# firedrakeproject/fiat

Hardware: AMD Instinct MI355X
Metric: element tabulations/sec (basis+grad, fp64) for batched P3 tet (higher is better)
Workload: dtype f64; 1 GPU; Lagrange degree 3 tetrahedron, order 1, 23 points/request, batch 100000 per GPU; requests_per_gpu=100000, points_per_request=23, order=1, points=random per request, world_size=1, launch=single process, clock_ramp_steps=224

## Files before the change

fiat_amd/csrc/api.hip:

```cpp
#include <hip/hip_runtime.h>

#include <algorithm>
#include <cmath>
#include <cstdarg>
#include <cstdio>
#include <cstring>
#include <cstdlib>
#include <mutex>
#include <string>
#include <thread>
#include <numeric>
#include <vector>

#include "../../include/fiat_amd.h"
#include "aux_kernels.hpp"
#include "plan.hpp"
#include "simplex_kernel.hpp"
#include "simplex_fixed.hpp"
#include "simplex_stream.hpp"
#include "simplex_pair.hpp"
#include "coop_kernel.hpp"
#include "shared_points.hpp"
#include "quadrature.hpp"
#include "simplex_small.hpp"
// ... 489 lines not shown

int fx_element_create(fx_ctx* ctx, int sd, int n, int variant, double scale, const double* verts,
                      int ndof, int vdim, const double* coeffs, fx_element** out) {
    if (!ctx || !out) return fail(FX_EINVAL, "fx_element_create: null argument");
    if (sd < 1 || sd > 3) return fail(FX_EINVAL, "Invalid number of spatial dimensions");
    if (n < 0) return fail(FX_EINVAL, "negative degree");
    if (variant < 0 || variant > 2) return fail(FX_EINVAL, "Invalid variant %d", variant);
    if (variant == FX_VARIANT_BUBBLE && n < 1) return fail(FX_EINVAL, "bubble variant needs degree >= 1");
    if (ndof < 1 || vdim < 1) return fail(FX_EINVAL, "bad ndof/vdim");
    HIP_TRY(hipSetDevice(ctx->device));
    fx_element* e = new fx_element;
    e->ctx = ctx;
    e->sd = sd;
    e->n = n;
    e->variant = variant;
    e->nexp = fx::binom(n + sd, sd);
    if (scale <= 0.0) {
        scale = std::sqrt(1.0 / default_simplex_volume(sd));
        if (n == 0 && sd > 1) scale = 1.0;
    }
    e->scale = scale;
    if (!host_cell_map(sd, verts ? verts : UFC[sd - 1], e->A0, e->b0)) {
        delete e;
        return fail(FX_EINVAL, "degenerate cell");
    }
    e->prog = fx::build_program(sd, n, variant, scale);
    if (variant == FX_VARIANT_BUBBLE) e->T = fx::c0_transform(sd, n);
    static_assert(sizeof(fx::Step) == sizeof(fxk::Step), "step layout");
    size_t sbytes = std::max<size_t>(1, e->prog.steps.size()) * sizeof(fxk::Step);
    hipError_t he = hipMalloc(&e->d_steps, sbytes);
    if (he == hipSuccess && !e->prog.steps.empty())
        he = hipMemcpy(e->d_steps, e->prog.steps.data(), e->prog.steps.size() * sizeof(fxk::Step), hipMemcpyHostToDevice);
    if (he != hipSuccess) {
        fx_element_destroy(e);
        return fail(FX_EHIP, "fx_element_create: %s", hipGetErrorString(he));
    }
    int rc = upload_coeffs(e, ndof, vdim, coeffs);
    if (rc != FX_OK) {
        fx_element_destroy(e);
        return rc;
    }
    *out = e;
    return FX_OK;
}

int fx_element_destroy(fx_element* e) {
    if (!e) return FX_OK;
    if (e->d_steps) (void)hipFree(e->d_steps);
    if (e->d_cmat) (void)hipFree(e->d_cmat);
    if (e->d_afrag) (void)hipFree(e->d_afrag);
    if (e->d_afrag_split) (void)hipFree(e->d_afrag_split);
    if (e->d_afrag_stream) (void)hipFree(e->d_afrag_stream);
    if (e->d_coop_eint) (void)hipFree(e->d_coop_eint);
    if (e->d_coop_edbl) (void)hipFree(e->d_coop_edbl);
    if (e->d_coop_kstart) (void)hipFree(e->d_coop_kstart);
    if (e->d_afrag_coop) (void)hipFree(e->d_afrag_coop);
    for (int o = 0; o < 3; ++o)
        if (e->d_astack[o]) (void)hipFree(e->d_astack[o]);
    for (int o = 0; o < 3; ++o) {
        if (e->d_astack_dm[o]) (void)hipFree(e->d_astack_dm[o]);
        if (e->d_astack_dmp[o]) (void)hipFree(e->d_astack_dmp[o]);
    }
    for (int o = 0; o <= FX_MAX_ORDER; ++o)
        if (e->high[o]) fx_element_destroy(e->high[o]);
    delete e;
    return FX_OK;
}

int fx_element_set_coeffs(fx_element* e, int ndof, int vdim, const double* coeffs) {
    if (!e || ndof < 1 || vdim < 1) return fail(FX_EINVAL, "fx_element_set_coeffs: bad argument");
    HIP_TRY(hipSetDevice(e->ctx->device));
    return upload_coeffs(e, ndof, vdim, coeffs);
}

int fx_element_dims(const fx_element* e, int* sd, int* n, int* nexp, int* ndof, int* vdim) {
    if (!e) return fail(FX_EINVAL, "fx_element_dims: null element");
    if (sd) *sd = e->sd;
    if (n) *n = e->n;
    if (nexp) *nexp = e->nexp;
    if (ndof) *ndof = e->ndof;
    if (vdim) *vdim = e->vdim;
    return FX_OK;
}

}

namespace {

struct Launch {
    fxk::TabArgs args;
    int grid = 0, lds_bytes = 0;
    int fixed_id = -1;
    fxk::FixedArgs<0> fhead;
    std::vector<double> fcoef;
    std::vector<double> fucoef;
    int fgrid = 0, flds_bytes = 0, ncu = 0;
    bool fused_mapping = false;
    bool kodd = false;
    int kpiola = 0;
    double* trash = nullptr;
    fx_ctx* ctx = nullptr;
    int fkind = 0;
    int small_id = -1;
    fxk::SmallArgs sargs;
    int sgrid = 0, slds_bytes = 0;
    int stacked_id = -1;
    fxk::StackedArgs<0> khead;
    int kgrid = 0, klds_bytes = 0, kmix_order = 0;
    int wg_ct = 0;
    int wg_mix = 0;
    int coop_id = -1;
    fxk::CoopArgs cargs;
    int cgrid = 0, clds_bytes = 0;
};

constexpr int FIXED_NW = 4;
struct FixedShape {
    int sd, n, order, rows, nt;
    bool pair_only;
    int rpw;
    bool fullimg;
    int nw;
    bool can_piola;
};
const FixedShape kFixedShapes[] = {
    {3, 3, 1, 20, 6, false, 2, true, 8, false},
    {3, 3, 1, 20, 5, true, 2, true, 8, false},
    {3, 3, 1, 20, 4, true, 2, true, 8, false},
    {3, 3, 1, 20, 3, true, 2, true, 8, false},
    {3, 3, 1, 20, 8, true, 1, false, 8, false},
    {3, 3, 1, 20, 10, true, 1, false, 8, false},
    {3, 3, 1, 20, 12, true, 1, false, 8, false},
    {3, 2, 1, 45, 6, true, 1, false, 8, true},
    {3, 4, 1, 35, 6, true, 1, false, 8, false},
    {3, 2, 1, 60, 6, true, 1, false, 4, true},
    {3, 3, 0, 20, 2, true, 2, true, 8, false},
    {3, 3, 0, 20, 3, true, 1, true, 8, false},
    {3, 4, 0, 35, 2, true, 2, true, 8, false},
    {3, 4, 0, 35, 3, true, 1, true, 8, false},
};

template <int SD, int N>
bool table_matches(const fx::Program& P) {
    constexpr fxk::StepTable<SD, N> T{};
    if ((int)P.steps.size() != T.count) return false;
    for (int i = 0; i < T.count; ++i)
        if (P.steps[i].dst != T.dst[i] || P.steps[i].cur != T.cur[i] || P.steps[i].prv != T.prv[i] ||
            P.steps[i].codim != T.codim[i])
            return false;
    return true;
}

#if defined(FX_DBG) && (FX_DBG & 512)
hipError_t report_wave_lifetimes(const double* trash, int grid, int wg_waves) {
    const int nw = std::min(grid * wg_waves, 3000);
    std::vector<double> t(2 * nw);
    hipError_t e = hipDeviceSynchronize();
    if (e != hipSuccess) return e;
    e = hipMemcpy(t.data(), trash + 2048, t.size() * 8, hipMemcpyDeviceToHost);
    if (e != hipSuccess) return e;
    std::vector<double> us(nw), mhz(nw);
    for (int i = 0; i < nw; ++i) {
        us[i] = t[2 * i + 1] / 100.0;
        mhz[i] = t[2 * i] / us[i];
    }
    std::vector<double> su = us, sm = mhz;
    std::sort(su.begin(), su.end());
    std::sort(sm.begin(), sm.end());
    fprintf(stderr, "[fiat_amd] %d waves: lifetime us min %.1f p10 %.1f median %.1f p90 %.1f max %.1f | clock MHz min %.0f median %.0f max %.0f\n",
            nw, su[0], su[nw / 10], su[nw / 2], su[nw * 9 / 10], su[nw - 1], sm[0], sm[nw / 2], sm[nw - 1]);
    for (int x = 0; x < 8; ++x) {
        std::vector<double> v;
        for (int i = 0; i < nw; ++i)
            if (((i / wg_waves) % 8) == x) v.push_back(us[i]);
        if (v.empty()) continue;
        std::sort(v.begin(), v.end());
        fprintf(stderr, " xcd%d %.0f..%.0f..%.0f", x, v[0], v[v.size() / 2], v.back());
    }
    {
        std::vector<double> ab(2 * nw), ini(nw);
        if (hipMemcpy(ab.data(), trash + 2048 + 6000, ab.size() * 8, hipMemcpyDeviceToHost) == hipSuccess &&
            hipMemcpy(ini.data(), trash + 2048 + 12000, ini.size() * 8, hipMemcpyDeviceToHost) == hipSuccess) {
            double t0 = 1e300, t1 = 0;
            for (int i = 0; i < nw; ++i) {
                t0 = std::min(t0, ab[2 * i]);
                t1 = std::max(t1, ab[2 * i + 1]);
            }
            std::vector<double> st(nw), en(nw);
            for (int i = 0; i < nw; ++i) {
                st[i] = (ab[2 * i] - t0) / 100.0;
                en[i] = (t1 - ab[2 * i + 1]) / 100.0;
            }
            std::vector<double> ss = st, se = en, si = ini;
            std::sort(ss.begin(), ss.end());
            std::sort(se.begin(), se.end());
            std::sort(si.begin(), si.end());
            fprintf(stderr, "\n span %.1f us | entry after first entry: p50 %.1f p90 %.1f max %.1f us | init->first unit: p50 %.1f max %.1f us | idle before the last exit: p10 %.1f p50 %.1f p90 %.1f max %.1f us (mean %.1f)",
                    (t1 - t0) / 100.0, ss[nw / 2], ss[nw * 9 / 10], ss[nw - 1], si[nw / 2] / 100.0, si[nw - 1] / 100.0, se[nw / 10], se[nw / 2],
                    se[nw * 9 / 10], se[nw - 1], std::accumulate(se.begin(), se.end(), 0.0) / nw);
            for (int x = 0; x < 8; ++x) {
                double ms = 0, me = 0;
                int n = 0;
                for (int i = 0; i < nw; ++i)
                    if (((i / wg_waves) % 8) == x) ms += st[i], me += en[i], ++n;
                if (n) fprintf(stderr, "%s xcd%d entry +%.1f idle-at-end %.1f", x == 0 ? "\n" : " |", x, ms / n, me / n);
            }
        }
    }
    fprintf(stderr, "\n workgroup lifetimes (max over its waves), XCD0:");
    for (int b = 0; b < grid; b += 8) {
        double m = 0;
        for (int w = 0; w < wg_waves && b * wg_waves + w < nw; ++w) m = std::max(m, us[b * wg_waves + w]);
        fprintf(stderr, " %.0f", m);
    }
    fprintf(stderr, "\n");
    return hipSuccess;
}
#endif

#ifndef FX_PAIR_BALANCE
#define FX_PAIR_BALANCE 0
#endif
template <int SD, int N, int ORDER, int ROWS, int NT, bool PAIR_ONLY = false, int RPW = 2, bool FULLIMG = true, int PAIR_NW = 8,
          bool CAN_PIOLA = false>
int launch_fixed(const Launch& L, hipStream_t s) {
    using KernT = void (*)(const fxk::FixedArgs<fxk::FixedNC<SD, N>::value>);
    constexpr int NC = fxk::FixedNC<SD, N>::value;
    fxk::FixedArgs<NC> fa;
    fa.pts = L.fhead.pts;
    fa.verts = L.fhead.verts;
    fa.out = L.fhead.out;
    fa.afrag = L.fhead.afrag;
    fa.phi0 = L.fhead.phi0;
    memcpy(fa.A0, L.fhead.A0, sizeof fa.A0);
    memcpy(fa.b0, L.fhead.b0, sizeof fa.b0);
    fa.nreq = L.fhead.nreq;
    fa.npts = L.fhead.npts;
    fa.lds_doubles = L.fhead.lds_doubles;
    fa.debug = L.fhead.debug;
    if ((int)L.fcoef.size() != NC || (int)L.fucoef.size() != 4 * NC)
        return fail(FX_EINVAL, "internal: coefficient table size mismatch");
    memcpy(fa.coef, L.fcoef.data(), NC * sizeof(double));
    memcpy(fa.ucoef, L.fucoef.data(), 4 * NC * sizeof(double));
    if (L.fkind == 2) {
        using KernP = void (*)(const fxk::FixedArgs<NC>, double*, unsigned int*);
        KernP kp = L.fhead.verts ? (KernP)fxk::tabulate_simplex_pair<SD, N, ORDER, ROWS, NT, PAIR_NW, false, RPW, FULLIMG>
                                 : (KernP)fxk::tabulate_simplex_pair<SD, N, ORDER, ROWS, NT, PAIR_NW, true, RPW, FULLIMG>;
        if ((fa.debug >> 16) & 3) {
            if constexpr (CAN_PIOLA) kp = (KernP)fxk::tabulate_simplex_pair<SD, N, ORDER, ROWS, NT, PAIR_NW, false, RPW, FULLIMG, true>;
            else return fail(FX_EINVAL, "internal: no fused push-forward for this shape");
        }
        const int lds_bytes = fxk::WQ_CTL_DOUBLES * 8 + (L.flds_bytes - (int)(fa.lds_doubles * 8) * FIXED_NW) + (int)(fa.lds_doubles * 8) * PAIR_NW;
        static thread_local const void* cached_kp = nullptr;
        static thread_local int cached_lds = -1, cached_occ = 0;
        if (cached_kp != reinterpret_cast<const void*>(kp) || cached_lds != lds_bytes) {
            if (lds_bytes > 48 * 1024)
                HIP_TRY(hipFuncSetAttribute(reinterpret_cast<const void*>(kp), hipFuncAttributeMaxDynamicSharedMemorySize, lds_bytes));
            int q = 0;
            HIP_TRY(hipOccupancyMaxActiveBlocksPerMultiprocessor(&q, reinterpret_cast<const void*>(kp), 64 * PAIR_NW, (size_t)lds_bytes));
            cached_kp = reinterpret_cast<const void*>(kp);
            cached_lds = lds_bytes;
            cached_occ = q;
        }
        const int occ = cached_occ;
        const long long nwg = ((L.fhead.nreq + RPW - 1) / RPW + PAIR_NW - 1) / PAIR_NW;
        int grid = (int)std::max<long long>(1, std::min<long long>(nwg, (long long)L.ncu * std::max(1, occ)));
#if FX_PAIR_BALANCE
        if (nwg > grid) {
            long long best = (nwg + grid - 1) / grid * grid - nwg;
            for (int g = grid - 1; g >= grid - grid / 8 && best > 0; --g) {
                const long long waste = (nwg + g - 1) / g * g - nwg;
                if (waste < best) {
                    best = waste;
                    grid = g;
                }
            }
        }
#endif
        static const bool verbose = ab_env("FIAT_AMD_VERBOSE") != nullptr;
        if (verbose) fprintf(stderr, "[fiat_amd] pair kernel: occupancy %d WG/CU, grid %d, lds %d B\n", occ, grid, lds_bytes);
        unsigned int* const counter = work_counter(L.ctx, s);
        if (!counter) return FX_ENOMEM;
        hipLaunchKernelGGL(kp, dim3(grid), dim3(64 * PAIR_NW), lds_bytes, s, fa, L.trash, counter);
        HIP_TRY(hipGetLastError());
#if defined(FX_DBG) && (FX_DBG & 512)
        if (verbose) HIP_TRY(report_wave_lifetimes(L.trash, grid, PAIR_NW));
#endif
        return FX_OK;
    }
    if constexpr (PAIR_ONLY) {
        return fail(FX_EINVAL, "internal: only the paired kernel exists for this shape");
    } else {
        KernT kern;
        if (L.fkind == 1)
            kern = L.fhead.verts ? (KernT)fxk::tabulate_simplex_stream<SD, N, ORDER, ROWS, NT, FIXED_NW, false>
                                 : (KernT)fxk::tabulate_simplex_stream<SD, N, ORDER, ROWS, NT, FIXED_NW, true>;
        else
            kern = (KernT)fxk::tabulate_simplex_fixed<SD, N, ORDER, ROWS, NT, FIXED_NW>;
        if (L.flds_bytes > 48 * 1024)
            HIP_TRY(hipFuncSetAttribute(reinterpret_cast<const void*>(kern), hipFuncAttributeMaxDynamicSharedMemorySize,
                                        L.flds_bytes));
        const int grid = L.fgrid;
        hipLaunchKernelGGL(kern, dim3(grid), dim3(64 * FIXED_NW), L.flds_bytes, s, fa);
        HIP_TRY(hipGetLastError());
        return FX_OK;
    }
}

struct StackedShape {
    int sd, n, ct, g;
    int rtc;
};
const StackedShape kStackedShapes[] = {
    {3, 3, 3, 2, 5},
    {3, 3, 2, 1, 5},
    {3, 3, 3, 1, 5},
    {3, 6, 2, 1, -2}, {3, 5, 3, 2, -2}, {3, 5, 2, 1, -2}, {3, 5, 3, 1, -2},
    {2, 6, 3, 2, -2}, {2, 6, 2, 1, -2}, {2, 6, 3, 1, -2}, {2, 5, 3, 2, -2}, {2, 5, 2, 1, -2}, {2, 5, 3, 1, -2},
    {3, 4, 3, 2, -2}, {3, 4, 2, 1, -2}, {3, 4, 3, 1, -2}, {3, 3, 3, 2, -2}, {3, 3, 2, 1, -2}, {3, 3, 3, 1, -2},
    {3, 6, 3, 2, 0},
    {3, 6, 2, 1, 0},
    {3, 6, 3, 1, 0},
    {3, 5, 3, 2, 0},
    {3, 5, 2, 1, 0},
    {3, 5, 3, 1, 0},
    {3, 4, 3, 2, 0},
    {3, 4, 2, 1, 0},
    {3, 4, 3, 1, 0},
    {3, 3, 3, 2, 0},
    {3, 3, 2, 1, 0},
    {3, 3, 3, 1, 0},
    {2, 6, 3, 2, 0},
    {2, 6, 2, 1, 0},
    {2, 6, 3, 1, 0},
    {2, 5, 3, 2, 0},
    {2, 5, 2, 1, 0},
    {2, 5, 3, 1, 0},
    {3, 6, 3, 3, 0},
    {3, 5, 3, 3, 0}, {3, 5, 4, 1, 0},
    {3, 4, 3, 3, 0}, {3, 4, 4, 1, 0},
    {3, 3, 3, 3, 0}, {3, 3, 4, 1, 0},
    {2, 6, 3, 3, 0}, {2, 6, 4, 1, 0},
    {2, 5, 3, 3, 0}, {2, 5, 4, 1, 0},
    {3, 2, 3, 2, 0}, {3, 2, 2, 1, 0}, {3, 2, 3, 1, 0}, {3, 2, 3, 3, 0}, {3, 2, 4, 1, 0},
    {3, 6, 3, 1, -1}, {3, 5, 3, 1, -1}, {3, 4, 3, 1, -1}, {3, 3, 3, 1, -1}, {3, 2, 3, 1, -1}, {2, 6, 3, 1, -1}, {2, 5, 3, 1, -1},
    {3, 2, 3, 4, 0},
    {2, 4, 3, 3, 0}, {2, 4, 3, 2, 0}, {2, 4, 2, 1, 0}, {2, 4, 3, 1, 0},
    {2, 3, 3, 4, 0}, {2, 3, 3, 3, 0}, {2, 3, 3, 2, 0}, {2, 3, 2, 1, 0},
    {3, 2, 3, 6, 0}, {3, 2, 3, 8, 0}, {3, 2, 3, 12, 0},
    {2, 3, 3, 6, 0}, {2, 3, 3, 8, 0}, {2, 4, 3, 4, 0}, {2, 4, 3, 6, 0},
    {2, 4, 3, 1, -1}, {2, 3, 3, 1, -1},
    {3, 2, 3, 4, -2}, {3, 2, 3, 3, -2}, {3, 2, 3, 2, -2}, {3, 2, 2, 1, -2},
    {2, 3, 3, 4, -2}, {2, 3, 3, 3, -2}, {2, 3, 3, 2, -2}, {2, 4, 3, 3, -2}, {2, 4, 3, 2, -2}, {2, 4, 2, 1, -2},
    {3, 7, 2, 1, 0}, {3, 7, 2, 1, -1},
    {2, 7, 3, 1, 0}, {2, 7, 2, 1, 0}, {2, 7, 3, 1, -1}, {2, 8, 4, 1, 0}, {2, 8, 3, 1, -1},
    {3, 2, 3, 4, -3}, {3, 2, 3, 3, -3}, {3, 2, 3, 2, -3}, {3, 2, 2, 1, -3},
    {3, 3, 3, 2, -3}, {3, 3, 2, 1, -3}, {3, 3, 3, 1, -3},
    {3, 4, 3, 2, -3}, {3, 4, 2, 1, -3}, {3, 4, 3, 1, -3},
    {3, 5, 2, 1, -3}, {3, 6, 2, 1, -3},
    {2, 3, 3, 4, -3}, {2, 3, 3, 3, -3}, {2, 3, 3, 2, -3},
    {2, 4, 3, 3, -3}, {2, 4, 3, 2, -3}, {2, 4, 2, 1, -3},
    {2, 5, 3, 2, -3}, {2, 5, 2, 1, -3}, {2, 5, 3, 1, -3},
    {2, 6, 3, 2, -3}, {2, 6, 2, 1, -3}, {2, 6, 3, 1, -3},
    {3, 6, 3, 2, -2}, {3, 6, 3, 1, -2},
    {3, 6, 3, 1, -4}, {3, 5, 3, 1, -4}, {3, 4, 3, 1, -4}, {3, 3, 3, 1, -4}, {3, 2, 3, 1, -4}, {2, 6, 3, 1, -4}, {2, 5, 3, 1, -4},
    {3, 6, 2, 1, -5}, {3, 5, 2, 1, -5}, {3, 4, 2, 1, -5}, {3, 3, 3, 1, -5}, {3, 2, 3, 1, -5}, {2, 6, 3, 1, -5}, {2, 5, 3, 1, -5},
    {3, 2, 3, 4, -6}, {3, 2, 3, 3, -6}, {3, 2, 3, 2, -6}, {3, 2, 2, 1, -6}, {3, 3, 3, 2, -6}, {3, 3, 2, 1, -6}, {3, 3, 3, 1, -6},
    {2, 3, 3, 4, -6}, {2, 3, 3, 3, -6}, {2, 3, 3, 2, -6}, {2, 4, 3, 3, -6}, {2, 4, 3, 2, -6}, {2, 4, 2, 1, -6},
    {3, 6, 2, 1, -1}, {3, 5, 2, 1, -1},
    {3, 6, 2, 1, -4}, {3, 5, 2, 1, -4},
    {3, 6, 8, 1, -7}, {3, 5, 8, 1, -7}, {3, 4, 8, 1, -7}, {3, 3, 8, 1, -7}, {2, 6, 8, 1, -7}, {2, 5, 8, 1, -7},
};
constexpr bool stacked_has_pio(int sd, int n) { return (sd == 3 && (n == 2 || n == 3)) || (sd == 2 && (n == 3 || n == 4)); }
constexpr int STACKED_NW = 4;
#ifndef FX_MIXR1
#define FX_MIXR1 1
#endif
constexpr bool mixr1(int sd, int n, int ct, int g) {
    return FX_MIXR1 == 2 || (FX_MIXR1 != 0 && !(sd == 2 && g == 1 && n == 4 && ct == 2));
}
constexpr int mixr_wps(int sd, int n) { return sd == 2 && n >= 5 ? 2 : 1; }
template <int SD>
int stacked_mix_pass(const Launch& L, hipStream_t s) {
    if (L.khead.verts && L.kmix_order >= 1) {
        fxk::TableMixArgs ma;
        ma.out = L.khead.out;
        ma.verts = L.khead.verts;
        if (!invert_small(SD, L.khead.A0, ma.A0inv)) return fail(FX_EINVAL, "degenerate cell");
        const int ntab = fx::binom(SD + L.kmix_order, SD);
        ma.n = L.khead.R / ntab * L.khead.npts;
        ma.order = L.kmix_order;
        ma.slices = std::max(1, std::min(8, (ma.n + 2047) / 2048));
        ma.nreq = L.khead.nreq;
        ma.rb = ma.n >= 1024 ? 1 : std::max(1, std::min(fxk::MIX_RB, 2048 / std::max(1, ma.n)));
        if (L.khead.nreq * ma.slices > 0x7fffffffLL) return fail(FX_EINVAL, "batch too large for the table-mixing pass");
        if ((long long)fxk::MIX_RB * ma.n > 0x3fffffffLL) return fail(FX_EINVAL, "request too large for the table-mixing pass");
        const long long blocks = ma.rb > 1 ? std::min<long long>((L.khead.nreq + ma.rb - 1) / ma.rb, (long long)L.ncu * 16) : L.khead.nreq * ma.slices;
        hipLaunchKernelGGL((fxk::table_mix_kernel<SD>), dim3((unsigned)std::max<long long>(1, blocks)), dim3(256), 0, s, ma);
        HIP_TRY(hipGetLastError());
    }
    return FX_OK;
}

template <int SD, int N, int CT, int G, int RTC = 0, int WPS = 1, bool CHUNK = false, int MIXT = 0, bool ODD = false, bool MIXR = false, int PIO = 0>
int launch_stacked(const Launch& L, hipStream_t s) {
    constexpr int NC = fxk::FixedNC<SD, N>::value;
    fxk::StackedArgs<NC> ka;
    ka.pts = L.khead.pts;
    ka.verts = L.khead.verts;
    ka.out = L.khead.out;
    ka.afrag = L.khead.afrag;
    ka.phi0 = L.khead.phi0;
    memcpy(ka.A0, L.khead.A0, sizeof ka.A0);
    memcpy(ka.b0, L.khead.b0, sizeof ka.b0);
    memcpy(ka.A0inv, L.khead.A0inv, sizeof ka.A0inv);
    memcpy(ka.G, L.khead.G, sizeof ka.G);
    ka.piola = L.khead.piola;
    ka.nreq = L.khead.nreq;
    ka.npts = L.khead.npts;
    ka.R = L.khead.R;
    ka.RT = L.khead.RT;
    ka.debug = L.khead.debug;
    ka.lim_pts = L.khead.lim_pts;
    ka.lim_verts = L.khead.lim_verts;
    ka.lim_out = L.khead.lim_out;
    ka.lim_afrag = L.khead.lim_afrag;
    if ((int)L.fcoef.size() != NC) return fail(FX_EINVAL, "internal: coefficient table size mismatch");
    memcpy(ka.coef, L.fcoef.data(), NC * sizeof(double));
    auto kern = fxk::tabulate_simplex_stacked<SD, N, CT, G, RTC, WPS, CHUNK, MIXT, ODD, MIXR, PIO>;
    static thread_local int occ = 0;
    if (occ == 0) {
        if (L.klds_bytes > 48 * 1024)
            HIP_TRY(hipFuncSetAttribute(reinterpret_cast<const void*>(kern), hipFuncAttributeMaxDynamicSharedMemorySize, L.klds_bytes));
        int q = 0;
        HIP_TRY(hipOccupancyMaxActiveBlocksPerMultiprocessor(&q, reinterpret_cast<const void*>(kern), 64 * STACKED_NW, (size_t)L.klds_bytes));
        occ = std::max(1, q);
        static const int cap = ab_env("FIAT_AMD_STACKED_WPS") ? atoi(ab_env("FIAT_AMD_STACKED_WPS")) : 8;
        occ = std::min(occ, std::max(1, cap));
        if (ab_env("FIAT_AMD_VERBOSE")) fprintf(stderr, "[fiat_amd] stacked kernel <%d,%d,%d,%d>: %d workgroups per CU, lds %d B\n", SD, N, CT, G, occ, L.klds_bytes);
// ... 2698 lines not shown
```

fiat_amd/csrc/simplex_pair.hpp:

```cpp
#pragma once
#include "simplex_stream.hpp"
#include "work_queue.hpp"

#ifndef FX_DBG
#define FX_DBG 0
#endif
#ifndef FX_PAIR_FULLIMG
#define FX_PAIR_FULLIMG 1
#endif
#ifndef FX_PAIR_PLAIN_EDGES
#define FX_PAIR_PLAIN_EDGES 1
#endif
#ifndef FX_PAIR_WAVES
#define FX_PAIR_WAVES 2
#endif

namespace fxk {

template <int SD, int N, int ORDER, int ROWS, int NT, int NW, bool UNIFORM, int RPW = 2, bool FULLIMG = (FX_PAIR_FULLIMG != 0),
          bool PIOLA = false>
__global__ __launch_bounds__(64 * NW, NW <= 4 ? 1 : FX_PAIR_WAVES) void tabulate_simplex_pair(const FixedArgs<FixedNC<SD, N>::value> a,
                                                                                double* __restrict__ trash,
                                                                                unsigned int* __restrict__ gqueue) {
    constexpr int NTAB = NTab<SD, ORDER>::value;
    constexpr StepTable<SD, N> TBL{};
    constexpr int NEXP = StepTable<SD, N>::NEXP;
    constexpr int KS = (NEXP + 3) / 4;
    constexpr int MT16 = rows_full16(ROWS);
    constexpr int M4 = rows_blk4(ROWS);
    static_assert(RPW == 1 || RPW == 2, "one or two requests per wave");
    static_assert(!PIOLA || (!UNIFORM && ROWS % SD == 0), "the Piola map needs per-request cells and SD components per dof");
    constexpr int NT2 = RPW * NT;
    extern __shared__ __attribute__((aligned(16))) double lds[];
    const int lane = threadIdx.x & 63;
    const int wave = __builtin_amdgcn_readfirstlane((int)(threadIdx.x >> 6));
#if FX_DBG & 512
    const unsigned long long rt_entry = __builtin_amdgcn_s_memrealtime();
#endif
    constexpr int NAF = (MT16 + M4) * KS;
    double* afr = lds + WQ_CTL_DOUBLES;
    double* img = afr + NAF * 64 + (size_t)wave * a.lds_doubles;
    double* slab = img;
    const int dump = a.lds_doubles - 64;

    typedef const __attribute__((address_space(4))) double CDouble;
    typedef FixedArgs<FixedNC<SD, N>::value> ArgsT;
    const __attribute__((address_space(4))) char* kargs =
        (const __attribute__((address_space(4))) char*)__builtin_amdgcn_kernarg_segment_ptr();
    CDouble* kcoef = (CDouble*)(kargs + __builtin_offsetof(ArgsT, coef));
    CDouble* kucoef = (CDouble*)(kargs + __builtin_offsetof(ArgsT, ucoef));

    const int npts = a.npts;
    double a0inv[SD][SD];
    if constexpr (PIOLA) {
        if constexpr (SD == 2) {
            const double det = a.A0[0] * a.A0[3] - a.A0[1] * a.A0[2];
            a0inv[0][0] = a.A0[3] / det;
            a0inv[0][1] = -a.A0[1] / det;
            a0inv[1][0] = -a.A0[2] / det;
            a0inv[1][1] = a.A0[0] / det;
        } else {
            const double* A = a.A0;
            const double c00 = A[4] * A[8] - A[5] * A[7], c01 = A[5] * A[6] - A[3] * A[8], c02 = A[3] * A[7] - A[4] * A[6];
            const double det = A[0] * c00 + A[1] * c01 + A[2] * c02;
            a0inv[0][0] = c00 / det;
            a0inv[0][1] = (A[2] * A[7] - A[1] * A[8]) / det;
            a0inv[0][2] = (A[1] * A[5] - A[2] * A[4]) / det;
            a0inv[1][0] = c01 / det;
            a0inv[1][1] = (A[0] * A[8] - A[2] * A[6]) / det;
            a0inv[1][2] = (A[2] * A[3] - A[0] * A[5]) / det;
            a0inv[2][0] = c02 / det;
            a0inv[2][1] = (A[1] * A[6] - A[0] * A[7]) / det;
            a0inv[2][2] = (A[0] * A[4] - A[1] * A[3]) / det;
        }
    }
    const int table = ROWS * npts;

    for (int i = lane; i < a.lds_doubles; i += 64) img[i] = 0.0;
    for (int i = threadIdx.x; i < NAF * 64; i += 64 * NW) afr[i] = a.afrag[i];
    const long long npairs = (a.nreq + RPW - 1) / RPW;
#ifndef FX_WQ_TAIL
#define FX_WQ_TAIL 0
#endif
    WorkQueueT<(FX_WQ_TAIL != 0)> wqueue;
    wqueue.init(lds, gqueue, npairs);
    __syncthreads();

    const int sub = RPW == 2 ? lane >> 5 : 0;
    const int lp = RPW == 2 ? lane & 31 : lane;
    const bool active = lp < npts;
    const int pl = active ? lp : 0;
    static_assert(FULLIMG || NT % 2 == 0 || NTAB == 1, "half-aligned column tiles need an even tile count");
    constexpr int TH = FULLIMG ? NTAB : (NTAB + 1) / 2;
    constexpr int NTH = NTAB > TH ? NT / 2 : NT;
    int colbase[NTAB];
#pragma unroll
    for (int t = 0; t < NTAB; ++t) {
        const int h = t >= TH ? 1 : 0;
        const int c = (t - h * TH) * npts + pl;
        colbase[t] = active ? (sub * NT + h * NTH + (c >> 4)) * 64 + (c & 15) : dump + (lane & 15);
    }
    constexpr int NFL = (TH * ROWS * ((16 * NTH) / TH) / 2 + 63) / 64;
    constexpr int NSTORE = RPW * NFL * (NTAB > TH ? 2 : 1);
    (void)NSTORE;
    int ioff[NT];
    {
        const float rinv = 1.0f / (float)npts;
#pragma unroll
        for (int nt = 0; nt < NT; ++nt) {
            const int h = nt / NTH;
            const int c = ((nt - h * NTH) << 4) + (lane & 15);
            const int ct = idiv_small(c, rinv);
            const int cp = c - ct * npts;
            const int nth = h == 0 ? TH : NTAB - TH;
            ioff[nt] = (ct < nth) ? ct * table + cp + (lane >> 4) * npts : -1;
        }
    }

    const long long phi = npairs;
    auto claim = [&]() -> long long { return wqueue.claim(); };
    long long pr = claim();
    wqueue.service();
    if (pr >= phi) {
        wqueue.finish();
        return;
    }
    long long pnext = claim();
#if FX_DBG & 512
    const unsigned long long clk0 = __builtin_readcyclecounter(), rt0 = rt_entry;
    const unsigned long long rt_first = __builtin_amdgcn_s_memrealtime();
#endif
    auto lane_req = [&](long long p) -> long long {
        long long r = RPW * p + sub;
        return r < a.nreq ? r : a.nreq - 1;
    };
    double xnext[SD];
    {
        const double* pp = a.pts + ((size_t)lane_req(pr) * npts + pl) * SD;
#pragma unroll
        for (int d = 0; d < SD; ++d) xnext[d] = pp[d];
    }
#pragma unroll
    for (int d = 0; d < SD; ++d) asm volatile("" : "+v"(xnext[d]));
    while (true) {
        double X[SD];
        double J[SD][SD];
        double Mreq[RPW][SD][SD];
        {
            double x[SD];
#pragma unroll
            for (int d = 0; d < SD; ++d) x[d] = xnext[d];
            {
                const long long pn = pnext < phi ? pnext : pr;
                const double* pp = a.pts + ((size_t)lane_req(pn) * npts + pl) * SD;
#pragma unroll
                for (int d = 0; d < SD; ++d) xnext[d] = pp[d];
            }
            double bb[SD];
            if constexpr (!UNIFORM) {
                cell_map<SD>(a.verts + (size_t)lane_req(pr) * (SD + 1) * SD, J, bb);
                if constexpr (PIOLA) {
                    const int kind = (a.debug >> 16) & 3;
#pragma unroll
                    for (int rq = 0; rq < RPW; ++rq) {
                        double Km[SD][SD];
#pragma unroll
                        for (int c = 0; c < SD; ++c)
#pragma unroll
                            for (int d = 0; d < SD; ++d) {
                                double t = 0.0;
#pragma unroll
                                for (int k = 0; k < SD; ++k) {
                                    const int lo = __builtin_amdgcn_readlane(__double2loint(J[k][d]), 32 * rq);
                                    const int hi = __builtin_amdgcn_readlane(__double2hiint(J[k][d]), 32 * rq);
                                    t += a0inv[c][k] * __hiloint2double(hi, lo);
                                }
                                Km[c][d] = t;
                            }
#pragma unroll
                        for (int c = 0; c < SD; ++c)
#pragma unroll
                            for (int e = 0; e < SD; ++e) {
                                double v = Km[e][c];
                                if (kind == 2) {
                                    if constexpr (SD == 2) v = (c == e ? Km[1 - c][1 - e] : -Km[c][e]);
                                    else if constexpr (SD == 3) {
                                        constexpr int nx[3] = {1, 2, 0}, nn[3] = {2, 0, 1};
                                        v = Km[nx[e]][nx[c]] * Km[nn[e]][nn[c]] - Km[nx[e]][nn[c]] * Km[nn[e]][nx[c]];
                                    }
                                }
                                Mreq[rq][c][e] = __hiloint2double(__builtin_amdgcn_readfirstlane(__double2hiint(v)),
                                                                  __builtin_amdgcn_readfirstlane(__double2loint(v)));
                            }
                    }
                }
#pragma unroll
                for (int i = 0; i < SD; ++i) {
                    double t = bb[i];
#pragma unroll
                    for (int d = 0; d < SD; ++d) t += J[i][d] * x[d];
                    X[i] = t;
                }
            } else {
#pragma unroll
                for (int i = 0; i < SD; ++i) {
                    double t = a.b0[i];
#pragma unroll
                    for (int d = 0; d < SD; ++d) t += a.A0[i * SD + d] * x[d];
                    X[i] = t;
                }
            }
        }

        v4d acc16[NT2][MT16 > 0 ? MT16 : 1];
        double acc4[NT2][M4 > 0 ? M4 : 1];

        Jet<SD, ORDER> mem[NEXP];
        Jet<SD, ORDER> zero;
        jet_zero(zero);
        Factors<SD, ORDER> F;
        double ufa = 0.0, ufb = 0.0, ufc = 0.0;
        int fcodim = -1;

        auto produce = [&](int slot) {
            if (slot == 0) {
                jet_zero(mem[0]);
                mem[0].v = a.phi0;
            } else if (FX_DBG & 1) {
                if (slot < NEXP) {
                    jet_zero(mem[TBL.dst[slot - 1]]);
                    mem[TBL.dst[slot - 1]].v = X[0];
                }
            } else if (slot < NEXP) {
                const int s = slot - 1;
                const CDouble* cb = kcoef;
                const CDouble* ub = kucoef;
                asm volatile("" : "+s"(cb), "+s"(ub));
                const CDouble* cp = cb + 3 * s;
                const CDouble* up = ub + 12 * s;
                const double cA = cp[0], cB = cp[1], cC = cp[2];
                if constexpr (UNIFORM) {
                    if (TBL.codim[s] != fcodim) {
                        fcodim = TBL.codim[s];
                        point_factors<SD>(fcodim, X, ufa, ufb, ufc);
                    }
                    apply_step_uniform<SD, ORDER>(mem[TBL.dst[s]], mem[TBL.cur[s]],
                                                  TBL.prv[s] < 0 ? zero : mem[TBL.prv[s]], ufa, ufb, ufc, cA, cB, cC,
                                                  up);
                } else {
                    if (TBL.codim[s] != fcodim) {
                        fcodim = TBL.codim[s];
                        make_factors<SD, ORDER>(F, fcodim, X, J);
                    }
                    apply_step<SD, ORDER>(mem[TBL.dst[s]], mem[TBL.cur[s]], TBL.prv[s] < 0 ? zero : mem[TBL.prv[s]],
                                          F, cA, cB, cC);
                }
            }
        };
        auto slot_jet = [&](int slot) -> const Jet<SD, ORDER>& {
            if (slot == 0) return mem[0];
            if (slot < NEXP) return mem[TBL.dst[slot - 1]];
            return zero;
        };
        auto put = [&](int kk, const Jet<SD, ORDER>& j) {
            if (FX_DBG & 8) return;
            slab[colbase[0] + kk * 16] = j.v;
            if constexpr (ORDER >= 1) {
#pragma unroll
                for (int d = 0; d < SD; ++d) slab[colbase[1 + d] + kk * 16] = j.g[d];
            }
            if constexpr (ORDER >= 2) {
#pragma unroll
                for (int h = 0; h < SD * (SD + 1) / 2; ++h) slab[colbase[1 + SD + h] + kk * 16] = j.h[h];
            }
        };

        int elane = lane;
        int eoff[NT];
        int enpts = npts;
        auto image_tile = [&](int rq, int nt) {
            const int so = eoff[nt];
            const bool mine = so >= 0;
            const int an = rq * NT + nt;
            const int dsink = dump + elane;
#pragma unroll
            for (int mt = 0; mt < MT16; ++mt) {
#pragma unroll
                for (int jj = 0; jj < 4; ++jj) {
                    const int mbase = 16 * mt + 4 * jj;
                    if (mbase + 3 < ROWS) {
                        img[mine ? so + mbase * enpts : dsink] = acc16[an][mt][jj];
                    } else if (mbase < ROWS) {
                        img[(mine && mbase + (elane >> 4) < ROWS) ? so + mbase * enpts : dsink] = acc16[an][mt][jj];
                    }
                }
            }
#pragma unroll
            for (int m4 = 0; m4 < M4; ++m4) {
                const int mbase = 16 * MT16 + 4 * m4;
                if (mbase + 3 < ROWS) {
                    img[mine ? so + mbase * enpts : dsink] = acc4[an][m4];
                } else {
                    img[(mine && mbase + (elane >> 4) < ROWS) ? so + mbase * enpts : dsink] = acc4[an][m4];
                }
            }
        };
        v2d carry = v2d{0.0, 0.0};
        auto flush_half = [&](long long req, int half) {
            const int ntab_h = half == 0 ? TH : NTAB - TH;
            const int nch = (ntab_h * ROWS * enpts) >> 1;
            const v2d* s2 = reinterpret_cast<const v2d*>(img);
            v2d* g2 = reinterpret_cast<v2d*>(a.out + (size_t)req * (NTAB * ROWS * enpts) + (size_t)half * TH * ROWS * enpts);
            constexpr int FB = 8;
            constexpr bool SHIFT = (ROWS * 8 * (FULLIMG ? NTAB : 1)) % 128 != 0;
            constexpr int NFLS = SHIFT ? NFL + 1 : NFL;
            int shift = 0;
            if constexpr (SHIFT) shift = (int)((reinterpret_cast<unsigned long long>(g2) >> 4) & 7ull);
            constexpr bool CARRY = SHIFT && !FULLIMG && NTAB > TH;
            int tl = 0, lo = 0;
            if constexpr (CARRY) {
                if (half == 0) tl = (shift + nch) & 7;
                else lo = -shift;
            }
            const int last = nch - 1 - tl;
#pragma unroll
            for (int b0 = 0; b0 < NFLS; b0 += FB) {
                v2d buf[FB];
#pragma unroll
                for (int it = b0; it < NFLS && it < b0 + FB; ++it) {
                    const int i = SHIFT ? max(0, min(it * 64 + elane - shift, last)) : min(it * 64 + elane, nch - 1);
                    buf[it - b0] = s2[i];
                    if constexpr (CARRY) {
                        if (it == 0 && half == 1 && elane < shift) buf[0] = carry;
                    }
                }
                if constexpr (CARRY) {
                    if (b0 == 0 && half == 0) carry = s2[min(nch - tl + elane, nch - 1)];
                }
#pragma unroll
                for (int it = b0; it < NFLS && it < b0 + FB; ++it) {
                    const int i = SHIFT ? max(lo, min(it * 64 + elane - shift, last)) : min(it * 64 + elane, nch - 1);
                    constexpr bool EDGES = FX_PAIR_PLAIN_EDGES && SHIFT && (NTAB * ROWS * 8) % 128 != 0;
                    if (EDGES && ((it == 0 && (!CARRY || half == 0)) || (it == NFLS - 1 && (!CARRY || half == 1)))) g2[i] = buf[it - b0];
                    else stream_store(&g2[i], buf[it - b0]);
                }
            }
        };

#pragma unroll
        for (int j = 0; j < KS; ++j) {
#pragma unroll
            for (int kk = 0; kk < 4; ++kk) produce(4 * j + kk);
#pragma unroll
            for (int kk = 0; kk < 4; ++kk) put(kk, slot_jet(4 * j + kk));
            wave_lds_fence();
            double a16[MT16 > 0 ? MT16 : 1], a4[M4 > 0 ? M4 : 1];
#pragma unroll
            for (int mt = 0; mt < MT16; ++mt) a16[mt] = afr[(mt * KS + j) * 64 + lane];
#pragma unroll
            for (int m4 = 0; m4 < M4; ++m4) a4[m4] = afr[((MT16 + m4) * KS + j) * 64 + lane];
#pragma unroll
            for (int rq = 0; rq < RPW; ++rq) {
                double b[NT];
#pragma unroll
                for (int nt = 0; nt < NT; ++nt) b[nt] = slab[(rq * NT + nt) * 64 + lane];
#pragma unroll
                for (int nt = 0; nt < NT; ++nt) {
                    const int an = rq * NT + nt;
                    if (FX_DBG & 2) {
                        acc4[an][0] += b[nt] * a4[0];
                        continue;
                    }
#pragma unroll
                    for (int mt = 0; mt < MT16; ++mt)
                        acc16[an][mt] = __builtin_amdgcn_mfma_f64_16x16x4f64(a16[mt], b[nt], j == 0 ? v4d{0.0, 0.0, 0.0, 0.0} : acc16[an][mt], 0, 0, 0);
#pragma unroll
                    for (int m4 = 0; m4 < M4; ++m4)
                        acc4[an][m4] = __builtin_amdgcn_mfma_f64_4x4x4f64(a4[m4], b[nt], j == 0 ? 0.0 : acc4[an][m4], 0, 0, 0);
                }
            }
            wave_lds_fence();
        }

        wqueue.service();
        const bool second = RPW * pr + 1 < a.nreq;
        elane = lane;
        asm volatile("" : "+v"(elane));
        enpts = npts;
        asm volatile("" : "+s"(enpts));
#pragma unroll
        for (int nt = 0; nt < NT; ++nt) {
            eoff[nt] = ioff[nt];
            asm volatile("" : "+v"(eoff[nt]));
        }
        if (!FX_ABL(a, 4)) {
            wave_lds_fence();
#pragma unroll
            for (int rq = 0; rq < RPW; ++rq) {
#pragma unroll
                for (int half = 0; half < (NTAB > TH ? 2 : 1); ++half) {
#pragma unroll
                    for (int nt = 0; nt < NTH; ++nt) image_tile(rq, half * NTH + nt);
                    wave_lds_fence();
                    if constexpr (PIOLA) {
                        double Mp[SD][SD];
#pragma unroll
                        for (int c = 0; c < SD; ++c)
#pragma unroll
                            for (int e = 0; e < SD; ++e) Mp[c][e] = Mreq[rq][c][e];
                        const float prinv = 1.0f / (float)enpts;
                        const int lb = idiv_small(elane, prinv), lq = elane - lb * enpts;
                        const int per = idiv_small(64, prinv);
                        const int nblk = (half == 0 ? TH : NTAB - TH) * (ROWS / SD);
                        for (int b0 = 0; b0 < nblk; b0 += per) {
                            const int b = b0 + lb;
                            const bool on = lb < per && b < nblk;
                            double* q = img + (on ? b * SD * enpts + lq : dump + elane);
                            double xin[SD];
#pragma unroll
                            for (int c = 0; c < SD; ++c) xin[c] = on ? q[c * enpts] : 0.0;
#pragma unroll
                            for (int c = 0; c < SD; ++c) {
                                double y = 0.0;
#pragma unroll
                                for (int e = 0; e < SD; ++e) y += Mp[c][e] * xin[e];
                                if (on) q[c * enpts] = y;
                            }
                        }
                        wave_lds_fence();
                    }
                    long long oreq = rq == 0 || second ? RPW * pr + rq : RPW * pr;
                    if (FX_DBG & 64) oreq &= 1023;
                    flush_half(oreq, half);
                    wave_lds_fence();
                }
            }
#pragma unroll
            for (int d = 0; d < SD; ++d) asm volatile("" : "+v"(xnext[d]));
        } else {
#pragma unroll
            for (int d = 0; d < SD; ++d) asm volatile("" : "+v"(xnext[d]));
        }
        if (pnext >= phi) break;
        pr = pnext;
        pnext = claim();
    }
    wqueue.service();
    wqueue.finish();
#if FX_DBG & 512
    if (lane == 0) {
        const long long gw = (long long)blockIdx.x * NW + wave;
        if (gw < 3000) {
            const unsigned long long rt1 = __builtin_amdgcn_s_memrealtime();
            trash[2048 + 2 * gw] = (double)(__builtin_readcyclecounter() - clk0);
            trash[2049 + 2 * gw] = (double)(rt1 - rt0);
            trash[2048 + 6000 + 2 * gw] = (double)(rt0 & 0xffffffffffffull);
            trash[2049 + 6000 + 2 * gw] = (double)(rt1 & 0xffffffffffffull);
            trash[2048 + 12000 + gw] = (double)(rt_first - rt0);
        }
    }
#endif
}

}
```

Before: 380.7 million tabulations/s.

## Defer work-queue claim and next-point prefetch to before the epilogue; enable tail queue

The paired tabulation kernel now claims its next work item and prefetches that item's points late in the current iteration, just before the store epilogue (configurable K-step position), instead of one item ahead at the start. The work queue's tail mode is also enabled by default. The intent is to reduce end-of-kernel load imbalance, since waves no longer hold a reserved item while finishing the current one, and to keep the point prefetch overlapped with the output flush. The cost is less latency hiding for the point load and queue claim, which now sit close to the point of use. Debug instrumentation for the time to first store is added as well.

Result: no change. 383.3 million tabulations/s, median of 5 (+0.7%).

```diff
diff --git a/fiat_amd/csrc/api.hip b/fiat_amd/csrc/api.hip
--- a/fiat_amd/csrc/api.hip
+++ b/fiat_amd/csrc/api.hip
@@ -665,7 +665,7 @@
 }
 
 #if defined(FX_DBG) && (FX_DBG & 512)
-hipError_t report_wave_lifetimes(const double* trash, int grid, int wg_waves) {
+hipError_t report_wave_lifetimes(const double* trash, int grid, int wg_waves, bool first_store = false) {
     const int nw = std::min(grid * wg_waves, 3000);
     std::vector<double> t(2 * nw);
     hipError_t e = hipDeviceSynchronize();
@@ -717,6 +717,12 @@
                 for (int i = 0; i < nw; ++i)
                     if (((i / wg_waves) % 8) == x) ms += st[i], me += en[i], ++n;
                 if (n) fprintf(stderr, "%s xcd%d entry +%.1f idle-at-end %.1f", x == 0 ? "\n" : " |", x, ms / n, me / n);
+            }
+            std::vector<double> fs(nw);
+            if (first_store && hipMemcpy(fs.data(), trash + 2048 + 15000, fs.size() * 8, hipMemcpyDeviceToHost) == hipSuccess) {
+                std::sort(fs.begin(), fs.end());
+                fprintf(stderr, "\n entry->first store: p50 %.1f p90 %.1f max %.1f us | first exit to last exit: %.1f us",
+                        fs[nw / 2] / 100.0, fs[nw * 9 / 10] / 100.0, fs[nw - 1] / 100.0, se[nw - 1]);
             }
         }
     }
@@ -797,7 +803,7 @@
         hipLaunchKernelGGL(kp, dim3(grid), dim3(64 * PAIR_NW), lds_bytes, s, fa, L.trash, counter);
         HIP_TRY(hipGetLastError());
 #if defined(FX_DBG) && (FX_DBG & 512)
-        if (verbose) HIP_TRY(report_wave_lifetimes(L.trash, grid, PAIR_NW));
+        if (verbose) HIP_TRY(report_wave_lifetimes(L.trash, grid, PAIR_NW, true));
 #endif
         return FX_OK;
     }
diff --git a/fiat_amd/csrc/simplex_pair.hpp b/fiat_amd/csrc/simplex_pair.hpp
--- a/fiat_amd/csrc/simplex_pair.hpp
+++ b/fiat_amd/csrc/simplex_pair.hpp
@@ -10,6 +10,9 @@
 #endif
 #ifndef FX_PAIR_PLAIN_EDGES
 #define FX_PAIR_PLAIN_EDGES 1
+#endif
+#ifndef FX_PAIR_CLAIM_AT
+#define FX_PAIR_CLAIM_AT KS
 #endif
 #ifndef FX_PAIR_WAVES
 #define FX_PAIR_WAVES 2
@@ -80,7 +83,7 @@
     for (int i = threadIdx.x; i < NAF * 64; i += 64 * NW) afr[i] = a.afrag[i];
     const long long npairs = (a.nreq + RPW - 1) / RPW;
 #ifndef FX_WQ_TAIL
-#define FX_WQ_TAIL 0
+#define FX_WQ_TAIL 1
 #endif
     WorkQueueT<(FX_WQ_TAIL != 0)> wqueue;
     wqueue.init(lds, gqueue, npairs);
@@ -117,6 +120,8 @@
         }
     }
 
+    constexpr int CLAIM_AT = (FX_PAIR_CLAIM_AT);
+    static_assert(CLAIM_AT >= 0 && CLAIM_AT <= KS, "claim position: before K-step 0 .. KS - 1, or KS = before the epilogue");
     const long long phi = npairs;
     auto claim = [&]() -> long long { return wqueue.claim(); };
     long long pr = claim();
@@ -125,10 +130,12 @@
         wqueue.finish();
         return;
     }
-    long long pnext = claim();
+    long long pnext = phi;
+    if constexpr (CLAIM_AT == 0) pnext = claim();
 #if FX_DBG & 512
     const unsigned long long clk0 = __builtin_readcyclecounter(), rt0 = rt_entry;
     const unsigned long long rt_first = __builtin_amdgcn_s_memrealtime();
+    unsigned long long rt_store = 0;
 #endif
     auto lane_req = [&](long long p) -> long long {
         long long r = RPW * p + sub;
@@ -142,6 +149,17 @@
     }
 #pragma unroll
     for (int d = 0; d < SD; ++d) asm volatile("" : "+v"(xnext[d]));
+    auto claim_next = [&]() {
+        wqueue.service();
+        pnext = claim();
+        wqueue.service();
+    };
+    auto fetch_next = [&]() {
+        const long long pn = pnext < phi ? pnext : pr;
+        const double* pp = a.pts + ((size_t)lane_req(pn) * npts + pl) * SD;
+#pragma unroll
+        for (int d = 0; d < SD; ++d) xnext[d] = pp[d];
+    };
     while (true) {
         double X[SD];
         double J[SD][SD];
@@ -150,12 +168,7 @@
             double x[SD];
 #pragma unroll
             for (int d = 0; d < SD; ++d) x[d] = xnext[d];
-            {
-                const long long pn = pnext < phi ? pnext : pr;
-                const double* pp = a.pts + ((size_t)lane_req(pn) * npts + pl) * SD;
-#pragma unroll
-                for (int d = 0; d < SD; ++d) xnext[d] = pp[d];
-            }
+            if constexpr (CLAIM_AT == 0) fetch_next();
             double bb[SD];
             if constexpr (!UNIFORM) {
                 cell_map<SD>(a.verts + (size_t)lane_req(pr) * (SD + 1) * SD, J, bb);
@@ -349,6 +362,12 @@
 
 #pragma unroll
         for (int j = 0; j < KS; ++j) {
+            if constexpr (CLAIM_AT > 0 && CLAIM_AT < KS) {
+                if (j == CLAIM_AT) {
+                    claim_next();
+                    fetch_next();
+                }
+            }
 #pragma unroll
             for (int kk = 0; kk < 4; ++kk) produce(4 * j + kk);
 #pragma unroll
@@ -383,6 +402,13 @@
         }
 
         wqueue.service();
+        if constexpr (CLAIM_AT == KS) {
+            claim_next();
+            fetch_next();
+        }
+#if FX_DBG & 512
+        if (rt_store == 0) rt_store = __builtin_amdgcn_s_memrealtime();
+#endif
         const bool second = RPW * pr + 1 < a.nreq;
         elane = lane;
         asm volatile("" : "+v"(elane));
@@ -443,7 +469,7 @@
         }
         if (pnext >= phi) break;
         pr = pnext;
-        pnext = claim();
+        if constexpr (CLAIM_AT == 0) pnext = claim();
     }
     wqueue.service();
     wqueue.finish();
@@ -457,6 +483,7 @@
             trash[2048 + 6000 + 2 * gw] = (double)(rt0 & 0xffffffffffffull);
             trash[2049 + 6000 + 2 * gw] = (double)(rt1 & 0xffffffffffffull);
             trash[2048 + 12000 + gw] = (double)(rt_first - rt0);
+            trash[2048 + 15000 + gw] = (double)(rt_store - rt0);
         }
     }
 #endif
```
